# chsakell/aca-dotnet-workshop

Hardware: AMD Instinct MI355X
Metric: tasks_e2e_per_sec (higher is better)
Workload: dtype n/a (JSON over HTTP)

## Files before the change

aca_dotnet_workshop_amd/native/src/applog.hpp:

```cpp
#pragma once

#include <fcntl.h>
#include <pthread.h>
#include <sys/stat.h>
#include <unistd.h>

#include <cerrno>
#include <algorithm>
#include <atomic>
#include <chrono>
#include <condition_variable>
#include <cstdint>
#include <cstdio>
#include <cstdlib>
#include <cstring>
#include <exception>
#include <functional>
#include <future>
#include <map>
#include <mutex>
#include <stdexcept>
#include <string>
#include <string_view>
#include <thread>
#include <vector>

namespace tt {

class AppLog {
 public:
  AppLog() = default;
  AppLog(const AppLog&) = delete;
  AppLog& operator=(const AppLog&) = delete;
  ~AppLog() {
    stop_committer();
    close();
  }

  bool open(const std::string& path, int fsync_mode) {
    path_ = path;
    fsync_ = fsync_mode;
    open_fd();
    if (fsync_ == 2 && !gc_thread_.joinable()) gc_thread_ = std::thread([this] { commit_loop(); });
    return true;
  }
  bool is_open() const { return fd_ >= 0; }
  uint64_t bytes() const { return bytes_; }
  const std::string& path() const { return path_; }

  void close() {
    std::lock_guard<std::mutex> f(fd_mu_);
    if (fd_ >= 0) { ::close(fd_); fd_ = -1; }
  }

  bool group() const { return fsync_ == 2 && fd_ >= 0; }
  uint64_t mark() const { return written_.load(std::memory_order_acquire); }
  void after_durable(uint64_t mark, std::function<void()> cb) {
    if (!group() || synced_.load(std::memory_order_acquire) >= mark) {
      cb();
      return;
    }
    {
      std::lock_guard<std::mutex> l(gc_mu_);
      waiters_.emplace(mark, std::move(cb));
      gc_want_ = true;
    }
    gc_cv_.notify_one();
  }
  void wait_durable(uint64_t mark) {
    if (!group() || synced_.load(std::memory_order_acquire) >= mark) return;
    std::promise<void> done;
    auto f = done.get_future();
    after_durable(mark, [&done] { done.set_value(); });
    f.wait();
  }
  void wait_durable() { wait_durable(mark()); }
  struct CommitStats {
    uint64_t syncs, acks, written, synced;
    double sync_ms_total, sync_ms_max;
  };
  CommitStats commit_stats() {
    std::lock_guard<std::mutex> l(gc_mu_);
    return {gc_syncs_, gc_acks_, mark(), synced_.load(), gc_sync_s_ * 1e3, gc_sync_max_s_ * 1e3};
  }

  static void put_field(std::string& rec, std::string_view f) {
    uint32_t n = (uint32_t)f.size();
    rec.append(reinterpret_cast<const char*>(&n), 4);
    rec.append(f.data(), f.size());
  }
  template <class T>
  static std::string_view pod(const T& v) { return std::string_view(reinterpret_cast<const char*>(&v), sizeof(T)); }

  void append(char kind, const std::vector<std::string_view>& fields) {
    if (fd_ < 0) return;
    std::string rec;
    rec.resize(5);
    rec[4] = kind;
    for (auto f : fields) put_field(rec, f);
    uint32_t total = (uint32_t)rec.size();
    std::memcpy(&rec[0], &total, 4);
    if (batching_) {
      batch_ += rec;
      return;
    }
    write_all(rec);
  }

  class BatchScope {
   public:
    explicit BatchScope(AppLog& log) : log_(log) { log_.batching_ = true; }
    ~BatchScope() noexcept(false) {
      log_.batching_ = false;
      if (log_.batch_.empty()) return;
      std::string b;
      b.swap(log_.batch_);
      if (std::uncaught_exceptions() == 0) {
        log_.write_all(b);
        return;
      }
      try {
        log_.write_all(b);
      } catch (...) {
      }
    }
    BatchScope(const BatchScope&) = delete;
    BatchScope& operator=(const BatchScope&) = delete;

   private:
    AppLog& log_;
  };

  void replay(const std::function<void(char, std::vector<std::string_view>&)>& fn) {
    if (fd_ < 0) return;
    std::string data;
    data.resize(bytes_);
// ... 32 lines not shown
  }

  void rewrite(const std::function<void(AppLog&)>& writer) {
    if (fd_ < 0) return;
    std::string tmp = path_ + ".compact";
    AppLog out;
    ::unlink(tmp.c_str());
    out.open(tmp, 0);
    writer(out);
    ::fdatasync(out.fd_);
    out.close();
    {
      std::lock_guard<std::mutex> f(fd_mu_);
      if (::rename(tmp.c_str(), path_.c_str()) != 0) throw std::runtime_error("log compaction rename failed");
      if (fd_ >= 0) ::close(fd_);
      fd_ = -1;
      open_fd_locked();
    }
    if (fsync_ == 2) {
      {
        std::lock_guard<std::mutex> l(gc_mu_);
        gc_want_ = true;
      }
      gc_cv_.notify_one();
    }
  }

  void sync() {
    std::lock_guard<std::mutex> f(fd_mu_);
    if (fd_ >= 0) ::fdatasync(fd_);
  }

 private:
  static FILE* stall_file(double& min_s) {
    static double th = [] {
      const char* p = std::getenv("TT_STALL_MS");
      double ms = p && *p ? std::atof(p) : 100.0;
      return (ms > 0 ? ms : 100.0) / 1e3;
    }();
    static FILE* f = [] {
      const char* p = std::getenv("TT_STALL_LOG");
      return p && *p ? std::fopen(p, "a") : nullptr;
    }();
    min_s = th;
    return f;
  }

  void write_all(const std::string& rec) {
    double min_s;
    FILE* stall = stall_file(min_s);
    auto t0 = stall ? std::chrono::steady_clock::now() : std::chrono::steady_clock::time_point{};
    size_t off = 0;
    while (off < rec.size()) {
      ssize_t w = ::write(fd_, rec.data() + off, rec.size() - off);
      if (w < 0) {
        if (errno == EINTR) continue;
        throw std::runtime_error(std::string("log write failed: ") + std::strerror(errno));
      }
      off += (size_t)w;
    }
    bytes_ += rec.size();
    written_.fetch_add(rec.size(), std::memory_order_release);
    if (fsync_ == 1) ::fdatasync(fd_);
    if (stall) {
      double s = std::chrono::duration<double>(std::chrono::steady_clock::now() - t0).count();
      if (s > min_s) {
        double wall = std::chrono::duration<double>(std::chrono::system_clock::now().time_since_epoch()).count();
        std::fprintf(stall, "{\"what\": \"log-write\", \"ms\": %.2f, \"bytes\": %zu, \"log\": \"%s\", \"pid\": %d, \"wall\": %.4f}\n",
                     s * 1e3, rec.size(), path_.c_str(), (int)::getpid(), wall);
        std::fflush(stall);
      }
    }
  }

  void open_fd() {
    std::lock_guard<std::mutex> f(fd_mu_);
    open_fd_locked();
  }
  void open_fd_locked() {
    fd_ = ::open(path_.c_str(), O_RDWR | O_CREAT | O_APPEND | O_CLOEXEC, 0644);
    if (fd_ < 0) throw std::runtime_error("cannot open log " + path_ + ": " + std::strerror(errno));
// ... 33 lines not shown
      for (auto it = waiters_.begin(); it != end; ++it) ready.push_back(std::move(it->second));
      waiters_.erase(waiters_.begin(), end);
      gc_acks_ += ready.size();
      if (!waiters_.empty()) gc_want_ = true;
      l.unlock();
      for (auto& f : ready) f();
      l.lock();
    }
  }
  void stop_committer() {
    if (!gc_thread_.joinable()) return;
    {
      std::lock_guard<std::mutex> l(gc_mu_);
      gc_stop_ = true;
      gc_want_ = true;
    }
    gc_cv_.notify_one();
    gc_thread_.join();
  }

  int fd_ = -1;
  int fsync_ = 0;
  uint64_t bytes_ = 0;
  std::string path_;
  bool batching_ = false;
  std::string batch_;
  std::mutex fd_mu_;
  std::atomic<uint64_t> written_{0}, synced_{0};
  std::mutex gc_mu_;
  std::condition_variable gc_cv_;
  std::multimap<uint64_t, std::function<void()>> waiters_;
  std::thread gc_thread_;
  bool gc_stop_ = false, gc_want_ = false;
  uint64_t gc_syncs_ = 0, gc_acks_ = 0;
  double gc_sync_s_ = 0, gc_sync_max_s_ = 0;
};

}
```

aca_dotnet_workshop_amd/native/src/docstore.hpp:

```cpp
#pragma once

#include <sys/random.h>

#include <algorithm>
#include <atomic>
#include <chrono>
#include <cmath>
#include <cstdint>
#include <map>
#include <memory>
#include <mutex>
#include <optional>
#include <string>
#include <thread>
#include <unordered_map>
#include <unordered_set>
#include <vector>

#include "applog.hpp"
#include "json.hpp"
#include "shardedmap.hpp"

namespace tt {

struct EtagMismatch : std::runtime_error {
  using std::runtime_error::runtime_error;
};
struct QueryError : std::runtime_error {
  using std::runtime_error::runtime_error;
};

inline int64_t now_ms() {
  return std::chrono::duration_cast<std::chrono::milliseconds>(std::chrono::system_clock::now().time_since_epoch()).count();
}

struct Filter {
  enum Op { ALL, EQ, NEQ, GT, GTE, LT, LTE, IN, AND, OR } op = ALL;
  std::string path;
  Value val;
  std::vector<Value> vals;
  std::vector<Filter> kids;
};

inline bool ieq(std::string_view a, const char* b) {
  size_t n = std::strlen(b);
// ... 112 lines not shown
  bool disabled = false;
  uint64_t gen = 1;
  std::vector<MirrorColumn> cols;
  std::vector<std::pair<const std::string, Doc>*> nodes;
  std::vector<int64_t> seqs;
  std::vector<uint8_t> live;
  std::vector<uint32_t> kills;
  size_t live_rows = 0;
  uint64_t compactions = 0;
};

struct MirrorDelta {
  uint64_t gen = 0;
  bool on = false, disabled = false, full = false;
  size_t n = 0, from = 0, kill_cursor = 0;
  std::vector<std::string> paths;
  std::vector<size_t> dict_from;
  std::vector<std::vector<std::string>> new_values;
  std::vector<std::vector<int32_t>> ids;
  std::vector<int64_t> seqs;
  std::vector<uint8_t> live;
  std::vector<uint32_t> kills;
};

struct TxOp {
  bool is_delete = false;
  std::string key;
  std::string value;
  std::optional<std::string> etag;
  bool first_write = false;
  int64_t ttl_ms = 0;
};

class DocStore {
 public:
  explicit DocStore(const std::string& path = "", int fsync_mode = 0, size_t index_threshold = 256)
      : index_threshold_(index_threshold) {
    if (!path.empty()) {
      log_.open(path, fsync_mode);
      log_.replay([this](char kind, std::vector<std::string_view>& f) { apply_log(kind, f); });
    }
  }

  std::string set(const std::string& key, const std::string& value, const std::optional<std::string>& etag,
                  bool first_write, int64_t ttl_ms) {
    Value parsed = parse(value);
    std::string text(value);
    std::vector<Doc> graveyard;
    std::lock_guard<std::mutex> g(mu_);
    int64_t now = now_ms();
    auto it = docs_.find(key);
    check_etag_at(it, etag, first_write, now);
    it = put_at(it, key, std::move(text), std::move(parsed), ttl_ms > 0 ? now + ttl_ms : 0, &graveyard);
    log_put(key, it->second.value, it->second.etag, it->second.expire_ms);
    maybe_compact();
    return std::to_string(it->second.etag);
  }

  struct BulkItem {
    std::string key, value;
    std::optional<std::string> etag;
    bool first_write = false;
    bool have_parsed = false;
    Value parsed;
  };
  struct BulkResult {
    std::string etag;
    int err = 0;
    std::string detail;
  };
  std::vector<BulkResult> set_many(std::vector<BulkItem>& items) {
    std::vector<BulkResult> out(items.size());
    for (size_t i = 0; i < items.size(); ++i) {
      if (items[i].have_parsed) continue;
      try {
        items[i].parsed = parse(items[i].value);
      } catch (const ParseError& e) {
        out[i].err = 2;
        out[i].detail = std::string("invalid JSON: ") + e.what();
      }
    }
    std::vector<Doc> graveyard;
    graveyard.reserve(items.size());
    {
      std::lock_guard<std::mutex> g(mu_);
      {
        AppLog::BatchScope batch(log_);
        const int64_t now = now_ms();
        for (size_t i = 0; i < items.size(); ++i) {
          if (out[i].err) continue;
          BulkItem& it = items[i];
          auto dit = docs_.find(it.key);
          const bool exists = dit != docs_.end() && !expired(dit->second, now);
          if (it.etag && !it.etag->empty()) {
            if (!exists || *it.etag != std::to_string(dit->second.etag)) {
              out[i].err = 1;
              out[i].detail = "possible etag mismatch";
              continue;
            }
          } else if (it.first_write && exists) {
            out[i].err = 1;
            out[i].detail = "possible etag mismatch: first-write on existing key without etag";
            continue;
          }
          dit = put_at(dit, it.key, std::move(it.value), std::move(it.parsed), 0, &graveyard);
          log_put(it.key, dit->second.value, dit->second.etag, dit->second.expire_ms);
          out[i].etag = std::to_string(dit->second.etag);
        }
      }
      maybe_compact();
    }
    return out;
  }

  std::optional<std::pair<std::string, std::string>> get(const std::string& key) {
    std::lock_guard<std::mutex> g(mu_);
    auto it = docs_.find(key);
    if (it == docs_.end()) return std::nullopt;
    if (expired(it->second, now_ms())) { erase_locked(key, true); return std::nullopt; }
    return std::make_pair(it->second.value, std::to_string(it->second.etag));
  }

  bool del(const std::string& key, const std::optional<std::string>& etag) {
    std::lock_guard<std::mutex> g(mu_);
    auto it = docs_.find(key);
    int64_t now = now_ms();
    if (it == docs_.end() || expired(it->second, now)) {
      if (etag && !etag->empty()) throw EtagMismatch("possible etag mismatch: key not found");
      return false;
    }
    if (etag && !etag->empty() && *etag != std::to_string(it->second.etag)) throw EtagMismatch("possible etag mismatch");
    erase_locked(key, true);
    maybe_compact();
    return true;
  }

  void transact(const std::vector<TxOp>& ops) {
    std::vector<Value> parsed(ops.size());
    for (size_t i = 0; i < ops.size(); ++i)
      if (!ops[i].is_delete) parsed[i] = parse(ops[i].value);
    std::lock_guard<std::mutex> g(mu_);
    int64_t now = now_ms();
    for (auto& op : ops) {
      if (op.is_delete) {
        if (op.etag && !op.etag->empty()) {
          auto it = docs_.find(op.key);
          if (it == docs_.end() || *op.etag != std::to_string(it->second.etag)) throw EtagMismatch("possible etag mismatch in transaction");
        }
      } else {
        check_etag(op.key, op.etag, op.first_write, now);
      }
    }
    log_.append('T', {std::string_view("begin")});
    for (size_t i = 0; i < ops.size(); ++i) {
      auto& op = ops[i];
      if (op.is_delete) {
        if (docs_.count(op.key)) erase_locked(op.key, true);
      } else {
        uint64_t e = put(op.key, op.value, std::move(parsed[i]), op.ttl_ms > 0 ? now + op.ttl_ms : 0);
        log_put(op.key, op.value, e, docs_[op.key].expire_ms);
      }
    }
    log_.append('T', {std::string_view("commit")});
    maybe_compact();
  }

  static void sort_keys_to(std::string& out, std::string_view key, const Doc& d, const std::vector<std::string>& paths) {
    out += "{\"key\":";
    escape_to(out, key);
    out += ",\"etag\":\"";
    out += std::to_string(d.etag);
    out += "\",\"sort\":[";
    for (size_t j = 0; j < paths.size(); ++j) {
      if (j) out += ',';
      const Value* v = d.parsed.path(paths[j]);
      if (v) dump_to(out, *v);
      else out += "null";
    }
    out += "]}";
  }

  std::string query(const std::string& query_json, const std::string& prefix, bool sort_keys = false) {
    Value q = parse(query_json.empty() ? std::string("{}") : query_json);
    if (q.t != Value::Object) throw QueryError("query must be a JSON object");
    Filter f;
    if (auto* fv = q.get_ci("filter")) f = compile_filter(*fv);
    std::vector<SortKey> sort;
    if (auto* sv = q.get_ci("sort")) {
      if (sv->t != Value::Array) throw QueryError("sort must be an array");
      for (auto& s : sv->items) {
        const Value* k = s.get_ci("key");
        if (!k || k->t != Value::String) throw QueryError("sort entry needs a string key");
        SortKey sk{k->s, false};
        if (auto* o = s.get_ci("order")) sk.desc = o->t == Value::String && ieq(o->s, "DESC");
        sort.push_back(sk);
      }
    }
    size_t limit = 0, offset = 0;
    if (auto* pv = q.get_ci("page")) {
      if (auto* l = pv->get_ci("limit")) limit = l->t == Value::Number && l->n > 0 ? (size_t)l->n : 0;
      if (auto* t = pv->get_ci("token")) {
        if (t->t == Value::String && !t->s.empty()) offset = (size_t)std::strtoull(t->s.c_str(), nullptr, 10);
      }
    }

    std::lock_guard<std::mutex> g(mu_);
    int64_t now = now_ms();
    ensure_indexes(f);
    std::vector<std::pair<const std::string*, const Doc*>> hits;
    auto consider = [&](const std::string& key, const Doc& d) {
      if (!prefix.empty() && key.compare(0, prefix.size(), prefix) != 0) return;
      if (expired(d, now)) return;
      if (!eval_filter(f, d.parsed)) return;
      hits.emplace_back(&key, &d);
    };
    std::unordered_set<std::string> cand;
    if (candidates(f, cand)) {
      ++stats_indexed_queries_;
      for (auto& k : cand) {
        auto it = docs_.find(k);
        if (it != docs_.end()) consider(it->first, it->second);
      }
    } else {
      ++stats_scan_queries_;
      for (auto& [k, d] : docs_) consider(k, d);
    }
    if (sort.empty()) {
      std::sort(hits.begin(), hits.end(), [](auto& a, auto& b) { return a.second->seq < b.second->seq; });
    } else {
      static const Value kNull;
      std::stable_sort(hits.begin(), hits.end(), [&](auto& a, auto& b) {
        for (auto& sk : sort) {
          const Value* x = a.second->parsed.path(sk.path);
          const Value* y = b.second->parsed.path(sk.path);
          int c = compare(x ? *x : kNull, y ? *y : kNull);
          if (c) return sk.desc ? c > 0 : c < 0;
        }
        return a.second->seq < b.second->seq;
      });
    }
    size_t begin = std::min(offset, hits.size());
    size_t end = limit ? std::min(hits.size(), begin + limit) : hits.size();
    std::string out = "{\"results\":[";
    std::vector<std::string> sort_paths;
    if (sort_keys)
      for (auto& sk : sort) sort_paths.push_back(sk.path);
    for (size_t i = begin; i < end; ++i) {
      if (i > begin) out += ',';
      if (sort_keys) {
        sort_keys_to(out, std::string_view(*hits[i].first).substr(prefix.size()), *hits[i].second, sort_paths);
        continue;
      }
      out += "{\"key\":";
      escape_to(out, std::string_view(*hits[i].first).substr(prefix.size()));
      out += ",\"data\":";
      out += hits[i].second->value;
      out += ",\"etag\":\"";
      out += std::to_string(hits[i].second->etag);
      out += "\"}";
    }
    out += "]";
    if (limit && end < hits.size()) {
      out += ",\"token\":\"" + std::to_string(end) + "\"";
    }
    out += "}";
    return out;
  }

  std::vector<std::string> keys(const std::string& prefix, size_t limit) {
    std::lock_guard<std::mutex> g(mu_);
    std::vector<std::pair<uint64_t, std::string>> ks;
    int64_t now = now_ms();
    for (auto& [k, d] : docs_)
      if ((prefix.empty() || k.compare(0, prefix.size(), prefix) == 0) && !expired(d, now)) ks.emplace_back(d.seq, k);
    std::sort(ks.begin(), ks.end());
    std::vector<std::string> out;
    for (auto& p : ks) { if (limit && out.size() >= limit) break; out.push_back(p.second); }
    return out;
  }

  struct EncodedColumn {
    std::vector<std::string> values;
    std::vector<int32_t> ids;
  };
  struct Encoded {
    std::string key_blob;
    std::vector<int64_t> key_off;
    std::vector<int64_t> seqs;
    std::vector<EncodedColumn> cols;
  };
  Encoded encode_columns(const std::string& prefix, const std::vector<std::string>& paths) {
    std::lock_guard<std::mutex> g(mu_);
    int64_t now = now_ms();
    std::vector<std::pair<uint64_t, const std::pair<const std::string, Doc>*>> rows;
    rows.reserve(docs_.size());
    for (auto& kv : docs_)
      if ((prefix.empty() || kv.first.compare(0, prefix.size(), prefix) == 0) && !expired(kv.second, now))
        rows.emplace_back(kv.second.seq, &kv);
    std::sort(rows.begin(), rows.end(), [](auto& a, auto& b) { return a.first < b.first; });
    Encoded out;
    out.key_off.reserve(rows.size() + 1);
    out.seqs.reserve(rows.size());
    out.key_off.push_back(0);
    for (auto& r : rows) {
      out.key_blob += r.second->first;
      out.key_off.push_back((int64_t)out.key_blob.size());
      out.seqs.push_back((int64_t)r.first);
    }
    out.cols.resize(paths.size());
    auto encode_one = [&](size_t c) {
      const std::string& path = paths[c];
      EncodedColumn& col = out.cols[c];
      col.ids.resize(rows.size());
      std::unordered_map<std::string, int32_t> dict;
      std::string k;
      for (size_t i = 0; i < rows.size(); ++i) {
        const std::string& key = rows[i].second->first;
        const Value& doc = rows[i].second->second.parsed;
        Value tmp;
        const Value* v;
        if (path == std::string("\x00keyprefix", 10)) {
          size_t p = key.find("||");
          tmp = Value::string(p == std::string::npos ? std::string() : key.substr(0, p + 2));
          v = &tmp;
        } else if (path == std::string("\x00value", 6)) {
// ... 106 lines not shown
    if (wait > kMaxReserveS) return std::max<int64_t>(1, (int64_t)std::ceil(wait * 1000.0));
    ru_tokens_ -= ru;
    do ticket_out = next_ticket();
    while (ru_tickets_.count(ticket_out));
    Reservation res{now + wait, ru, bind};
    ru_tickets_.emplace(ticket_out, res);
    ru_by_slot_.emplace(res.slot, ticket_out);
    if (bind) ru_by_bind_.emplace(bind, ticket_out);
    return std::max<int64_t>(1, (int64_t)std::ceil(wait * 1000.0));
  }

  void debit(double ru) {
    std::lock_guard<std::mutex> g(ru_mu_);
    ru_consumed_ += ru;
    if (ru_rate_ <= 0) return;
    double now = mono_s();
    ru_tokens_ = std::min(ru_rate_, ru_tokens_ + (now - ru_last_) * ru_rate_) - ru;
    ru_last_ = now;
  }

  std::unordered_map<std::string, double> throughput_stats() {
    std::lock_guard<std::mutex> g(ru_mu_);
    return {{"ru_per_s", ru_rate_}, {"ru_consumed", ru_consumed_}, {"throttled", (double)ru_throttled_},
            {"reserved_admits", (double)ru_reserved_admits_}, {"open_reservations", (double)ru_tickets_.size()},
            {"calls", (double)ru_calls_}, {"early_retries", (double)ru_early_retries_},
            {"lapsed_reservations", (double)ru_lapsed_}, {"refunded_ru", ru_refunded_},
            {"throttled_read", (double)ru_throttled_kind_[kRead]}, {"throttled_write", (double)ru_throttled_kind_[kWrite]},
            {"throttled_query", (double)ru_throttled_kind_[kQuery]},
            {"throttled_delete", (double)ru_throttled_kind_[kDelete]},
            {"mono", mono_s()}};
  }

  bool mirror_enable(const std::vector<std::string>& paths) {
    std::lock_guard<std::mutex> g(mu_);
    if (mirror_.disabled) return false;
    std::vector<std::string> add;
    for (auto& p : paths) {
      bool have = false;
      for (auto& c : mirror_.cols) have = have || c.path == p;
      for (auto& a : add) have = have || a == p;
      if (!have) add.push_back(p);
    }
    if (mirror_.on && add.empty()) return true;
    if (!mirror_.on) {
      for (auto& [k, d] : docs_)
        if (d.expire_ms) { mirror_.disabled = true; return false; }
      mirror_.on = true;
      mirror_.cols.clear();
      for (auto& p : add) { mirror_.cols.emplace_back(); mirror_.cols.back().path = p; }
      mirror_rebuild_rows();
    } else {
      size_t first = mirror_.cols.size();
      for (auto& p : add) { mirror_.cols.emplace_back(); mirror_.cols.back().path = p; }
      auto enc = [&](size_t c) {
        MirrorColumn& col = mirror_.cols[c];
        col.ids.assign(mirror_.nodes.size(), -1);
        std::string k;
        for (size_t r = 0; r < mirror_.nodes.size(); ++r) {
          if (!mirror_.live[r]) continue;
          auto& kv = *mirror_.nodes[r];
          col.ids[r] = mirror_encode(col, kv.first, kv.second.parsed, k);
        }
      };
      parallel_for_columns(first, mirror_.cols.size(), enc);
      ++mirror_.gen;
      mirror_.kills.clear();
    }
    return true;
  }

  MirrorDelta mirror_delta(uint64_t gen, size_t from, size_t kill_from, const std::vector<size_t>& dict_sizes) {
    std::lock_guard<std::mutex> g(mu_);
    MirrorDelta d;
    d.gen = mirror_.gen;
    d.on = mirror_.on;
    d.disabled = mirror_.disabled;
    if (!mirror_.on) return d;
    size_t n = mirror_.nodes.size();
    d.full = gen != mirror_.gen || dict_sizes.size() != mirror_.cols.size() || from > n ||
             kill_from > mirror_.kills.size();
    if (d.full) from = 0, kill_from = mirror_.kills.size();
    d.n = n;
    d.from = from;
    d.kill_cursor = mirror_.kills.size();
    for (size_t i = kill_from; i < mirror_.kills.size(); ++i)
      if (mirror_.kills[i] < from) d.kills.push_back(mirror_.kills[i]);
    d.seqs.assign(mirror_.seqs.begin() + from, mirror_.seqs.end());
    d.live.assign(mirror_.live.begin() + from, mirror_.live.end());
    for (size_t c = 0; c < mirror_.cols.size(); ++c) {
      auto& col = mirror_.cols[c];
      size_t df = d.full ? 0 : std::min(dict_sizes[c], col.values.size());
      d.paths.push_back(col.path);
      d.dict_from.push_back(df);
      d.new_values.emplace_back(col.values.begin() + df, col.values.end());
      d.ids.emplace_back(col.ids.begin() + from, col.ids.end());
    }
    return d;
  }

  bool mirror_results(const int32_t* rows, size_t nrows, const std::string& prefix, const std::string& token,
                      uint64_t gen, std::string& out, size_t* skipped = nullptr,
                      const std::vector<std::string>* sort_paths = nullptr) {
    std::lock_guard<std::mutex> g(mu_);
    if (gen != mirror_.gen) return false;
    int64_t now = now_ms();
    out.clear();
    if (!sort_paths && !docs_.empty()) out.reserve(32 + token.size() + nrows * (live_bytes_ / docs_.size() + 48));
    out += "{\"results\":[";
    size_t skip = 0;
    bool first = true;
    for (size_t i = 0; i < nrows; ++i) {
      uint32_t r = (uint32_t)rows[i];
      if (r >= mirror_.nodes.size() || !mirror_.live[r]) { ++skip; continue; }
      auto* it = mirror_.nodes[r];
      const std::string& key = it->first;
      if (it->second.mrow != r || expired(it->second, now)) { ++skip; continue; }
      if (!first) out += ',';
      first = false;
      if (sort_paths) {
        sort_keys_to(out, std::string_view(key).substr(std::min(prefix.size(), key.size())), it->second, *sort_paths);
        continue;
      }
      out += "{\"key\":";
      escape_to(out, std::string_view(key).substr(std::min(prefix.size(), key.size())));
      out += ",\"data\":";
      out += it->second.value;
      out += ",\"etag\":\"";
      out += std::to_string(it->second.etag);
      out += "\"}";
    }
    out += "]";
    if (!token.empty()) out += ",\"token\":\"" + token + "\"";
    out += "}";
    if (skipped) *skipped = skip;
    return true;
  }

  std::unordered_map<std::string, uint64_t> mirror_stats() {
    std::lock_guard<std::mutex> g(mu_);
    return {{"on", mirror_.on}, {"disabled", mirror_.disabled}, {"gen", mirror_.gen},
            {"rows", mirror_.nodes.size()}, {"live_rows", mirror_.live_rows}, {"columns", mirror_.cols.size()},
            {"compactions", mirror_.compactions}};
  }

  size_t size() {
    std::lock_guard<std::mutex> g(mu_);
    return docs_.size();
  }

  void compact() {
    std::lock_guard<std::mutex> g(mu_);
    compact_locked();
  }

  void sync() { std::lock_guard<std::mutex> g(mu_); log_.sync(); }
  bool group_commit() const { return log_.group(); }
  uint64_t log_mark() const { return log_.mark(); }
  void after_durable(uint64_t mark, std::function<void()> cb) { log_.after_durable(mark, std::move(cb)); }
  void wait_durable() { log_.wait_durable(); }
  AppLog::CommitStats commit_stats() { return log_.commit_stats(); }

  std::unordered_map<std::string, uint64_t> stats() {
    std::lock_guard<std::mutex> g(mu_);
    return {{"docs", docs_.size()}, {"live_bytes", live_bytes_}, {"log_bytes", log_.bytes()},
            {"indexes", indexes_.size()}, {"indexed_queries", stats_indexed_queries_},
            {"scan_queries", stats_scan_queries_}, {"etag", etag_}};
  }

  std::vector<std::string> indexed_paths() {
    std::lock_guard<std::mutex> g(mu_);
    std::vector<std::string> out;
    for (auto& [p, _] : indexes_) out.push_back(p);
    std::sort(out.begin(), out.end());
    return out;
  }

 private:
  using Index = std::unordered_map<std::string, std::unordered_set<std::string>>;
  using Docs = ShardedMap<Doc>;

  static bool expired(const Doc& d, int64_t now) { return d.expire_ms && d.expire_ms <= now; }

  void check_etag(const std::string& key, const std::optional<std::string>& etag, bool first_write, int64_t now) {
    check_etag_at(docs_.find(key), etag, first_write, now);
  }

  void check_etag_at(Docs::iterator it, const std::optional<std::string>& etag,
                     bool first_write, int64_t now) {
    bool exists = it != docs_.end() && !expired(it->second, now);
    if (etag && !etag->empty()) {
      if (!exists || *etag != std::to_string(it->second.etag)) throw EtagMismatch("possible etag mismatch");
    } else if (first_write && exists) {
      throw EtagMismatch("possible etag mismatch: first-write on existing key without etag");
    }
  }

  uint64_t put(const std::string& key, const std::string& value, Value parsed, int64_t expire_ms) {
    return put_at(docs_.find(key), key, std::string(value), std::move(parsed), expire_ms, nullptr)->second.etag;
  }

  static bool same_scalar(const Value* a, const Value* b) {
    if (!a || !b) return a == b;
    if (a->t != b->t) return false;
    switch (a->t) {
      case Value::Null: return true;
      case Value::Bool: return a->b == b->b;
      case Value::Number: return std::memcmp(&a->n, &b->n, sizeof(double)) == 0;
      case Value::String: return a->s == b->s;
      default: return false;
    }
  }

  Docs::iterator put_at(Docs::iterator it,
                                                       const std::string& key, std::string&& value, Value parsed,
                                                       int64_t expire_ms, std::vector<Doc>* graveyard) {
    uint64_t e = ++etag_;
    if (expire_ms && mirror_.on) mirror_disable();
    int32_t* reuse = nullptr;
    if (it == docs_.end()) {
      Doc d;
      live_bytes_ += key.size() + value.size();
      d.value = std::move(value);
      d.parsed = std::move(parsed);
      d.etag = e;
      d.seq = ++seq_;
      d.expire_ms = expire_ms;
      index_add(key, d.parsed);
      it = docs_.emplace(key, std::move(d)).first;
    } else {
      Doc& d = it->second;
      index_update(key, d.parsed, parsed);
      if (mirror_.on && d.mrow < mirror_.live.size() && mirror_.live[d.mrow]) {
        reuse_.resize(mirror_.cols.size());
        for (size_t c = 0; c < mirror_.cols.size(); ++c)
          reuse_[c] = same_column_value(mirror_.cols[c], d.parsed, parsed) ? mirror_.cols[c].ids[d.mrow] : kEncode;
        reuse = reuse_.data();
      }
      live_bytes_ += value.size();
      live_bytes_ -= d.value.size();
      if (graveyard) {
        graveyard->emplace_back();
        graveyard->back().value.swap(d.value);
        graveyard->back().parsed = std::move(d.parsed);
// ... 39 lines not shown
      erase_locked(std::string(f[0]), false);
    }
  }

  void maybe_compact() {
    if (!log_.is_open()) return;
    uint64_t live = live_bytes_ + docs_.size() * 40;
    if (log_.bytes() > (1u << 20) && log_.bytes() > 4 * live) compact_locked();
  }

  void compact_locked() {
    if (!log_.is_open()) return;
    std::vector<std::pair<uint64_t, const std::pair<const std::string, Doc>*>> rows;
    for (auto& kv : docs_) rows.emplace_back(kv.second.seq, &kv);
    std::sort(rows.begin(), rows.end(), [](auto& a, auto& b) { return a.first < b.first; });
    log_.rewrite([&](AppLog& out) {
      for (auto& r : rows)
        out.append('P', {r.second->first, r.second->second.value, AppLog::pod(r.second->second.etag),
                         AppLog::pod(r.second->second.expire_ms)});
    });
  }

  template <class F>
  void parallel_for_columns(size_t lo, size_t hi, F&& f) {
    if (hi - lo <= 1 || mirror_.nodes.size() < 100000) {
      for (size_t c = lo; c < hi; ++c) f(c);
      return;
    }
    std::vector<std::thread> ts;
    for (size_t c = lo; c < hi; ++c) ts.emplace_back(f, c);
    for (auto& t : ts) t.join();
  }

  static int32_t mirror_encode(MirrorColumn& col, const std::string& key, const Value& doc, std::string& k) {
    static const std::string kPrefix("\x00keyprefix", 10), kValue("\x00value", 6);
    Value tmp;
    const Value* v;
    if (col.path == kPrefix) {
      size_t p = key.find("||");
      tmp = Value::string(p == std::string::npos ? std::string() : key.substr(0, p + 2));
      v = &tmp;
    } else if (col.path == kValue) {
      v = doc.t == Value::Object ? nullptr : &doc;
    } else {
      v = doc.path(col.path);
    }
    if (!v) return -1;
    mirror_key(*v, k);
    auto it = col.dict.find(k);
    if (it == col.dict.end()) {
      it = col.dict.emplace(k, (int32_t)col.values.size()).first;
      col.values.push_back(dump(*v));
    }
    return it->second;
  }

  static bool same_column_value(const MirrorColumn& col, const Value& before, const Value& after) {
    static const std::string kPrefix("\x00keyprefix", 10), kValue("\x00value", 6);
    if (col.path == kPrefix) return true;
    if (col.path == kValue)
      return before.t != Value::Object && after.t != Value::Object && same_scalar(&before, &after);
    return same_scalar(before.path(col.path), after.path(col.path));
  }

  void mirror_append(std::pair<const std::string, Doc>& kv, const int32_t* reuse = nullptr) {
    uint32_t r = (uint32_t)mirror_.nodes.size();
    mirror_.nodes.push_back(&kv);
    mirror_.seqs.push_back((int64_t)kv.second.seq);
    mirror_.live.push_back(1);
    std::string k;
    for (size_t c = 0; c < mirror_.cols.size(); ++c) {
      MirrorColumn& col = mirror_.cols[c];
      col.ids.push_back(reuse && reuse[c] != kEncode ? reuse[c] : mirror_encode(col, kv.first, kv.second.parsed, k));
    }
    kv.second.mrow = r;
    ++mirror_.live_rows;
    if (mirror_.nodes.size() > 65536 && mirror_.nodes.size() > 2 * mirror_.live_rows) mirror_compact();
  }

  void mirror_kill(Doc& d) {
    if (d.mrow == UINT32_MAX) return;
    if (mirror_.on && d.mrow < mirror_.live.size() && mirror_.live[d.mrow]) {
      mirror_.live[d.mrow] = 0;
      mirror_.kills.push_back(d.mrow);
      --mirror_.live_rows;
    }
    d.mrow = UINT32_MAX;
  }

  void mirror_disable() {
    for (auto& kv : docs_) kv.second.mrow = UINT32_MAX;
    uint64_t gen = mirror_.gen;
    mirror_ = ColumnMirror{};
    mirror_.gen = gen + 1;
    mirror_.disabled = true;
  }

  void mirror_rebuild_rows() {
    std::vector<std::pair<uint64_t, std::pair<const std::string, Doc>*>> rows;
    rows.reserve(docs_.size());
    for (auto& kv : docs_) rows.emplace_back(kv.second.seq, &kv);
    std::sort(rows.begin(), rows.end(), [](auto& a, auto& b) { return a.first < b.first; });
    mirror_.nodes.clear();
    mirror_.seqs.clear();
    mirror_.kills.clear();
    mirror_.nodes.reserve(rows.size());
    for (auto& r : rows) {
// ... 11 lines not shown
        col.ids[i] = mirror_encode(col, rows[i].second->first, rows[i].second->second.parsed, k);
    };
    parallel_for_columns(0, mirror_.cols.size(), enc);
    ++mirror_.gen;
  }

  void mirror_compact() {
    size_t w = 0, n = mirror_.nodes.size();
    for (size_t r = 0; r < n; ++r) {
      if (!mirror_.live[r]) continue;
      if (w != r) {
        mirror_.nodes[w] = mirror_.nodes[r];
        mirror_.seqs[w] = mirror_.seqs[r];
        for (auto& col : mirror_.cols) col.ids[w] = col.ids[r];
        mirror_.nodes[w]->second.mrow = (uint32_t)w;
      }
      ++w;
    }
    mirror_.nodes.resize(w);
    mirror_.seqs.resize(w);
    for (auto& col : mirror_.cols) col.ids.resize(w);
    mirror_.live.assign(w, 1);
    mirror_.live_rows = w;
    mirror_.kills.clear();
    ++mirror_.gen;
    ++mirror_.compactions;
  }

  void collect_eq_paths(const Filter& f, std::vector<std::string>& out) {
    if (f.op == Filter::EQ || f.op == Filter::IN) out.push_back(f.path);
    for (auto& k : f.kids) collect_eq_paths(k, out);
  }

  void ensure_indexes(const Filter& f) {
    if (docs_.size() < index_threshold_) return;
    std::vector<std::string> paths;
    collect_eq_paths(f, paths);
    for (auto& p : paths) {
      if (indexes_.count(p)) continue;
      Index& idx = indexes_[p];
      for (auto& [k, d] : docs_) {
        const Value* v = d.parsed.path(p);
        if (v && v->t != Value::Array && v->t != Value::Object) idx[index_key(*v)].insert(k);
      }
    }
  }

  void index_add(const std::string& key, const Value& doc) {
    for (auto& [p, idx] : indexes_) {
      const Value* v = doc.path(p);
      if (v && v->t != Value::Array && v->t != Value::Object) idx[index_key(*v)].insert(key);
    }
  }

  void index_update(const std::string& key, const Value& before, const Value& after) {
    for (auto& [p, idx] : indexes_) {
      const Value* a = before.path(p);
      const Value* b = after.path(p);
      if (same_scalar(a, b)) continue;
      if (a && a->t != Value::Array && a->t != Value::Object) {
        auto it = idx.find(index_key(*a));
        if (it != idx.end()) {
          it->second.erase(key);
          if (it->second.empty()) idx.erase(it);
        }
      }
// ... 23 lines not shown
        return true;
      }
      case Filter::IN: {
        auto ix = indexes_.find(f.path);
        if (ix == indexes_.end()) return false;
        for (auto& v : f.vals) {
          if (v.t == Value::Array || v.t == Value::Object) return false;
          auto it = ix->second.find(index_key(v));
          if (it != ix->second.end()) out.insert(it->second.begin(), it->second.end());
        }
        return true;
      }
      case Filter::AND: {
        bool any = false;
        std::unordered_set<std::string> best;
        for (auto& k : f.kids) {
          std::unordered_set<std::string> c;
          if (candidates(k, c) && (!any || c.size() < best.size())) { best.swap(c); any = true; }
        }
        if (any) out.insert(best.begin(), best.end());
        return any;
      }
      case Filter::OR: {
        std::unordered_set<std::string> acc;
        for (auto& k : f.kids)
          if (!candidates(k, acc)) return false;
        out.insert(acc.begin(), acc.end());
        return true;
      }
      default: return false;
    }
  }

  std::mutex mu_;
  Docs docs_;
  std::unordered_map<std::string, Index> indexes_;
  AppLog log_;
  uint64_t etag_ = 0;
  uint64_t seq_ = 0;
  uint64_t live_bytes_ = 0;
  uint64_t stats_indexed_queries_ = 0;
  uint64_t stats_scan_queries_ = 0;
  size_t index_threshold_;
  ColumnMirror mirror_;
  static constexpr int32_t kEncode = INT32_MIN;
  std::vector<int32_t> reuse_;
  std::mutex ru_mu_;
  std::atomic<bool> ru_on_{false};
  double ru_rate_ = 0, ru_tokens_ = 0, ru_last_ = 0, ru_consumed_ = 0;
  uint64_t ru_throttled_ = 0, ru_reserved_admits_ = 0, ru_calls_ = 0, ru_early_retries_ = 0, ru_lapsed_ = 0;
  uint64_t ru_throttled_kind_[4] = {0, 0, 0, 0};
  double ru_refunded_ = 0;
  double ru_ticket_ttl_s_ = kTicketTtlS;
  struct Reservation {
    double slot, ru;
    uint64_t bind;
  };
  std::unordered_map<uint64_t, Reservation> ru_tickets_;
  std::multimap<double, uint64_t> ru_by_slot_;
  std::unordered_multimap<uint64_t, uint64_t> ru_by_bind_;
  uint64_t ru_rng_[2] = {0, 0};
  uint64_t next_ticket() {
    if ((ru_rng_[0] | ru_rng_[1]) == 0) {
      if (getrandom(ru_rng_, sizeof ru_rng_, 0) != (ssize_t)sizeof ru_rng_ || (ru_rng_[0] | ru_rng_[1]) == 0)
        ru_rng_[0] = 0x9e3779b97f4a7c15ull ^ (uint64_t)(mono_s() * 1e9);
    }
    uint64_t a = ru_rng_[0];
    const uint64_t b = ru_rng_[1];
    ru_rng_[0] = b;
    a ^= a << 23;
    ru_rng_[1] = a ^ b ^ (a >> 17) ^ (b >> 26);
    uint64_t v = (ru_rng_[1] + b) >> 1;
    return v ? v : 1;
  }
  void drop(std::unordered_map<uint64_t, Reservation>::iterator it) {
// ... 36 lines not shown
```

Before: 87220.

## Replace store mutex with rwlock and split bulk writes into shared prepare and exclusive commit

The document store's mutex becomes a writer-preferring pthread rwlock. Reads (get, queries with existing indexes, mirror results, stats) take a shared lock, and set_many now precomputes index ops, mirror column ids and encoded log records under shared locks in slices. The exclusive section then only applies the prepared plan, falling back to the old path when a version or shape has changed. Mirror result emission gains prefetching, and the log gets an append-encoded path. This aims to cut time spent holding the exclusive lock, at the cost of more complexity, double lookups and rwlock overhead on short critical sections.

Measured after the change: 87140. Within noise of the previous version (-0.1%).

```diff
diff --git a/aca_dotnet_workshop_amd/native/src/applog.hpp b/aca_dotnet_workshop_amd/native/src/applog.hpp
--- a/aca_dotnet_workshop_amd/native/src/applog.hpp
+++ b/aca_dotnet_workshop_amd/native/src/applog.hpp
@@ -56,7 +56,7 @@
   bool group() const { return fsync_ == 2 && fd_ >= 0; }
   uint64_t mark() const { return written_.load(std::memory_order_acquire); }
   void after_durable(uint64_t mark, std::function<void()> cb) {
-    if (!group() || synced_.load(std::memory_order_acquire) >= mark) {
+    if (!group() || covered(mark)) {
       cb();
       return;
     }
@@ -68,7 +68,7 @@
     gc_cv_.notify_one();
   }
   void wait_durable(uint64_t mark) {
-    if (!group() || synced_.load(std::memory_order_acquire) >= mark) return;
+    if (!group() || covered(mark)) return;
     std::promise<void> done;
     auto f = done.get_future();
     after_durable(mark, [&done] { done.set_value(); });
@@ -81,7 +81,7 @@
   };
   CommitStats commit_stats() {
     std::lock_guard<std::mutex> l(gc_mu_);
-    return {gc_syncs_, gc_acks_, mark(), synced_.load(), gc_sync_s_ * 1e3, gc_sync_max_s_ * 1e3};
+    return {gc_syncs_, gc_acks_.load(), mark(), synced_.load(), gc_sync_s_ * 1e3, gc_sync_max_s_ * 1e3};
   }
 
   static void put_field(std::string& rec, std::string_view f) {
@@ -92,16 +92,27 @@
   template <class T>
   static std::string_view pod(const T& v) { return std::string_view(reinterpret_cast<const char*>(&v), sizeof(T)); }
 
+  static size_t encode(std::string& out, char kind, const std::vector<std::string_view>& fields) {
+    const size_t at = out.size();
+    out.resize(at + 5);
+    out[at + 4] = kind;
+    for (auto f : fields) put_field(out, f);
+    uint32_t total = (uint32_t)(out.size() - at);
+    std::memcpy(&out[at], &total, 4);
+    return at;
+  }
+
   void append(char kind, const std::vector<std::string_view>& fields) {
     if (fd_ < 0) return;
     std::string rec;
-    rec.resize(5);
-    rec[4] = kind;
-    for (auto f : fields) put_field(rec, f);
-    uint32_t total = (uint32_t)rec.size();
-    std::memcpy(&rec[0], &total, 4);
+    encode(rec, kind, fields);
+    append_encoded(rec);
+  }
+
+  void append_encoded(std::string_view rec) {
+    if (fd_ < 0) return;
     if (batching_) {
-      batch_ += rec;
+      batch_.append(rec.data(), rec.size());
       return;
     }
     write_all(rec);
@@ -200,6 +211,12 @@
   }
 
  private:
+  bool covered(uint64_t mark) {
+    if (synced_.load(std::memory_order_acquire) < mark) return false;
+    gc_acks_.fetch_add(1, std::memory_order_relaxed);
+    return true;
+  }
+
   static FILE* stall_file(double& min_s) {
     static double th = [] {
       const char* p = std::getenv("TT_STALL_MS");
@@ -214,7 +231,7 @@
     return f;
   }
 
-  void write_all(const std::string& rec) {
+  void write_all(std::string_view rec) {
     double min_s;
     FILE* stall = stall_file(min_s);
     auto t0 = stall ? std::chrono::steady_clock::now() : std::chrono::steady_clock::time_point{};
@@ -314,7 +331,8 @@
   std::multimap<uint64_t, std::function<void()>> waiters_;
   std::thread gc_thread_;
   bool gc_stop_ = false, gc_want_ = false;
-  uint64_t gc_syncs_ = 0, gc_acks_ = 0;
+  uint64_t gc_syncs_ = 0;
+  std::atomic<uint64_t> gc_acks_{0};
   double gc_sync_s_ = 0, gc_sync_max_s_ = 0;
 };
 
diff --git a/aca_dotnet_workshop_amd/native/src/docstore.hpp b/aca_dotnet_workshop_amd/native/src/docstore.hpp
--- a/aca_dotnet_workshop_amd/native/src/docstore.hpp
+++ b/aca_dotnet_workshop_amd/native/src/docstore.hpp
@@ -1,5 +1,6 @@
 #pragma once
 
+#include <pthread.h>
 #include <sys/random.h>
 
 #include <algorithm>
@@ -7,10 +8,12 @@
 #include <chrono>
 #include <cmath>
 #include <cstdint>
+#include <functional>
 #include <map>
 #include <memory>
 #include <mutex>
 #include <optional>
+#include <shared_mutex>
 #include <string>
 #include <thread>
 #include <unordered_map>
@@ -189,7 +192,33 @@
   int64_t ttl_ms = 0;
 };
 
+class RwLock {
+ public:
+  RwLock() {
+    pthread_rwlockattr_t a;
+    pthread_rwlockattr_init(&a);
+#ifdef PTHREAD_RWLOCK_PREFER_WRITER_NONRECURSIVE_NP
+    pthread_rwlockattr_setkind_np(&a, PTHREAD_RWLOCK_PREFER_WRITER_NONRECURSIVE_NP);
+#endif
+    pthread_rwlock_init(&l_, &a);
+    pthread_rwlockattr_destroy(&a);
+  }
+  ~RwLock() { pthread_rwlock_destroy(&l_); }
+  RwLock(const RwLock&) = delete;
+  RwLock& operator=(const RwLock&) = delete;
+  void lock() { pthread_rwlock_wrlock(&l_); }
+  void unlock() { pthread_rwlock_unlock(&l_); }
+  void lock_shared() { pthread_rwlock_rdlock(&l_); }
+  void unlock_shared() { pthread_rwlock_unlock(&l_); }
+
+ private:
+  pthread_rwlock_t l_;
+};
+
 class DocStore {
+  using Exclusive = std::lock_guard<RwLock>;
+  using Shared = std::shared_lock<RwLock>;
+
  public:
   explicit DocStore(const std::string& path = "", int fsync_mode = 0, size_t index_threshold = 256)
       : index_threshold_(index_threshold) {
@@ -204,7 +233,7 @@
     Value parsed = parse(value);
     std::string text(value);
     std::vector<Doc> graveyard;
-    std::lock_guard<std::mutex> g(mu_);
+    Exclusive g(mu_);
     int64_t now = now_ms();
     auto it = docs_.find(key);
     check_etag_at(it, etag, first_write, now);
@@ -227,51 +256,93 @@
     std::string detail;
   };
   std::vector<BulkResult> set_many(std::vector<BulkItem>& items) {
+    using clk = std::chrono::steady_clock;
+    auto ns = [](clk::time_point a, clk::time_point b) {
+      return (uint64_t)std::chrono::duration_cast<std::chrono::nanoseconds>(b - a).count();
+    };
     std::vector<BulkResult> out(items.size());
-    for (size_t i = 0; i < items.size(); ++i) {
-      if (items[i].have_parsed) continue;
-      try {
-        items[i].parsed = parse(items[i].value);
-      } catch (const ParseError& e) {
-        out[i].err = 2;
-        out[i].detail = std::string("invalid JSON: ") + e.what();
-      }
-    }
+    parse_items(items, out);
+    std::vector<Doc> graveyard;
+    graveyard.reserve(items.size());
+    std::vector<uint64_t> etags(items.size(), 0);
+    BulkPlan plan;
+    uint64_t prepare_ns = 0;
+    for (size_t from = 0; from < items.size(); from += kPrepareSlice) {
+      Shared s(mu_);
+      const auto t0 = clk::now();
+      const bool go_on = prepare_bulk(items, out, plan, from, std::min(items.size(), from + kPrepareSlice));
+      prepare_ns += ns(t0, clk::now());
+      if (!go_on) break;
+    }
+    bulk_prepare_us_.fetch_add(prepare_ns / 1000, std::memory_order_relaxed);
+    if (bulk_gap_hook_) bulk_gap_hook_();
+    {
+      Exclusive g(mu_);
+      const auto t0 = clk::now();
+      {
+        AppLog::BatchScope batch(log_);
+        const int64_t now = now_ms();
+        const bool same_shape = plan.mirror_on == mirror_.on && plan.ncols == mirror_.cols.size() &&
+                                plan.nindexes == indexes_.size();
+        uint64_t prepared = 0, fallback = 0;
+        for (size_t i = 0; i < items.size(); ++i) {
+          if (out[i].err) continue;
+          ++prepared;
+          auto dit = docs_.find(items[i].key);
+          const uint64_t version = dit == docs_.end() ? 0 : dit->second.etag;
+          if (same_shape && version == plan.items[i].seen) {
+            etags[i] = commit_prepared(dit, items[i], out[i], plan, i, now, graveyard);
+          } else {
+            ++fallback;
+            etags[i] = bulk_put_locked(dit, items[i], out[i], now, graveyard);
+          }
+        }
+        bulk_prepared_.fetch_add(prepared, std::memory_order_relaxed);
+        bulk_fallback_.fetch_add(fallback, std::memory_order_relaxed);
+      }
+      maybe_compact();
+      bulk_hold_us_.fetch_add(ns(t0, clk::now()) / 1000, std::memory_order_relaxed);
+    }
+    for (size_t i = 0; i < items.size(); ++i)
+      if (etags[i]) out[i].etag = std::to_string(etags[i]);
+    return out;
+  }
+
+  std::vector<BulkResult> set_many_serial(std::vector<BulkItem>& items) {
+    std::vector<BulkResult> out(items.size());
+    parse_items(items, out);
     std::vector<Doc> graveyard;
     graveyard.reserve(items.size());
     {
-      std::lock_guard<std::mutex> g(mu_);
+      Exclusive g(mu_);
+      const auto t0 = std::chrono::steady_clock::now();
       {
         AppLog::BatchScope batch(log_);
         const int64_t now = now_ms();
         for (size_t i = 0; i < items.size(); ++i) {
           if (out[i].err) continue;
-          BulkItem& it = items[i];
-          auto dit = docs_.find(it.key);
-          const bool exists = dit != docs_.end() && !expired(dit->second, now);
-          if (it.etag && !it.etag->empty()) {
-            if (!exists || *it.etag != std::to_string(dit->second.etag)) {
-              out[i].err = 1;
-              out[i].detail = "possible etag mismatch";
-              continue;
-            }
-          } else if (it.first_write && exists) {
-            out[i].err = 1;
-            out[i].detail = "possible etag mismatch: first-write on existing key without etag";
-            continue;
-          }
-          dit = put_at(dit, it.key, std::move(it.value), std::move(it.parsed), 0, &graveyard);
-          log_put(it.key, dit->second.value, dit->second.etag, dit->second.expire_ms);
-          out[i].etag = std::to_string(dit->second.etag);
+          if (uint64_t e = bulk_put_locked(docs_.find(items[i].key), items[i], out[i], now, graveyard))
+            out[i].etag = std::to_string(e);
         }
       }
       maybe_compact();
+      bulk_hold_us_.fetch_add(
+          (uint64_t)std::chrono::duration_cast<std::chrono::microseconds>(std::chrono::steady_clock::now() - t0).count(),
+          std::memory_order_relaxed);
     }
     return out;
   }
 
+  void set_bulk_gap_hook(std::function<void()> hook) { bulk_gap_hook_ = std::move(hook); }
+
   std::optional<std::pair<std::string, std::string>> get(const std::string& key) {
-    std::lock_guard<std::mutex> g(mu_);
+    {
+      Shared s(mu_);
+      auto it = docs_.find(key);
+      if (it == docs_.end()) return std::nullopt;
+      if (!expired(it->second, now_ms())) return std::make_pair(it->second.value, std::to_string(it->second.etag));
+    }
+    Exclusive g(mu_);
     auto it = docs_.find(key);
     if (it == docs_.end()) return std::nullopt;
     if (expired(it->second, now_ms())) { erase_locked(key, true); return std::nullopt; }
@@ -279,7 +350,7 @@
   }
 
   bool del(const std::string& key, const std::optional<std::string>& etag) {
-    std::lock_guard<std::mutex> g(mu_);
+    Exclusive g(mu_);
     auto it = docs_.find(key);
     int64_t now = now_ms();
     if (it == docs_.end() || expired(it->second, now)) {
@@ -296,7 +367,7 @@
     std::vector<Value> parsed(ops.size());
     for (size_t i = 0; i < ops.size(); ++i)
       if (!ops[i].is_delete) parsed[i] = parse(ops[i].value);
-    std::lock_guard<std::mutex> g(mu_);
+    Exclusive g(mu_);
     int64_t now = now_ms();
     for (auto& op : ops) {
       if (op.is_delete) {
@@ -361,9 +432,19 @@
       }
     }
 
-    std::lock_guard<std::mutex> g(mu_);
+    {
+      Shared s(mu_);
+      if (!missing_index(f)) return query_locked(f, sort, limit, offset, prefix, sort_keys);
+    }
+    Exclusive g(mu_);
+    ensure_indexes(f);
+    return query_locked(f, sort, limit, offset, prefix, sort_keys);
+  }
+
+ private:
+  std::string query_locked(const Filter& f, const std::vector<SortKey>& sort, size_t limit, size_t offset,
+                           const std::string& prefix, bool sort_keys) {
     int64_t now = now_ms();
-    ensure_indexes(f);
     std::vector<std::pair<const std::string*, const Doc*>> hits;
     auto consider = [&](const std::string& key, const Doc& d) {
       if (!prefix.empty() && key.compare(0, prefix.size(), prefix) != 0) return;
@@ -373,13 +454,13 @@
     };
     std::unordered_set<std::string> cand;
     if (candidates(f, cand)) {
-      ++stats_indexed_queries_;
+      stats_indexed_queries_.fetch_add(1, std::memory_order_relaxed);
       for (auto& k : cand) {
         auto it = docs_.find(k);
         if (it != docs_.end()) consider(it->first, it->second);
       }
     } else {
-      ++stats_scan_queries_;
+      stats_scan_queries_.fetch_add(1, std::memory_order_relaxed);
       for (auto& [k, d] : docs_) consider(k, d);
     }
     if (sort.empty()) {
@@ -424,8 +505,9 @@
     return out;
   }
 
+ public:
   std::vector<std::string> keys(const std::string& prefix, size_t limit) {
-    std::lock_guard<std::mutex> g(mu_);
+    Exclusive g(mu_);
     std::vector<std::pair<uint64_t, std::string>> ks;
     int64_t now = now_ms();
     for (auto& [k, d] : docs_)
@@ -447,7 +529,7 @@
     std::vector<EncodedColumn> cols;
   };
   Encoded encode_columns(const std::string& prefix, const std::vector<std::string>& paths) {
-    std::lock_guard<std::mutex> g(mu_);
+    Exclusive g(mu_);
     int64_t now = now_ms();
     std::vector<std::pair<uint64_t, const std::pair<const std::string, Doc>*>> rows;
     rows.reserve(docs_.size());
@@ -620,7 +702,7 @@
   }
 
   bool mirror_enable(const std::vector<std::string>& paths) {
-    std::lock_guard<std::mutex> g(mu_);
+    Exclusive g(mu_);
     if (mirror_.disabled) return false;
     std::vector<std::string> add;
     for (auto& p : paths) {
@@ -658,7 +740,7 @@
   }
 
   MirrorDelta mirror_delta(uint64_t gen, size_t from, size_t kill_from, const std::vector<size_t>& dict_sizes) {
-    std::lock_guard<std::mutex> g(mu_);
+    Shared g(mu_);
     MirrorDelta d;
     d.gen = mirror_.gen;
     d.on = mirror_.on;
@@ -689,7 +771,7 @@
   bool mirror_results(const int32_t* rows, size_t nrows, const std::string& prefix, const std::string& token,
                       uint64_t gen, std::string& out, size_t* skipped = nullptr,
                       const std::vector<std::string>* sort_paths = nullptr) {
-    std::lock_guard<std::mutex> g(mu_);
+    Shared g(mu_);
     if (gen != mirror_.gen) return false;
     int64_t now = now_ms();
     out.clear();
@@ -697,7 +779,16 @@
     out += "{\"results\":[";
     size_t skip = 0;
     bool first = true;
+    constexpr size_t kAhead = 8;
+    auto live_node = [&](size_t i) -> const std::pair<const std::string, Doc>* {
+      uint32_t r = (uint32_t)rows[i];
+      return r < mirror_.nodes.size() && mirror_.live[r] ? mirror_.nodes[r] : nullptr;
+    };
     for (size_t i = 0; i < nrows; ++i) {
+      if (i + kAhead < nrows)
+        if (auto* n = live_node(i + kAhead)) __builtin_prefetch(&n->second);
+      if (i + kAhead / 2 < nrows)
+        if (auto* n = live_node(i + kAhead / 2)) __builtin_prefetch(n->second.value.data());
       uint32_t r = (uint32_t)rows[i];
       if (r >= mirror_.nodes.size() || !mirror_.live[r]) { ++skip; continue; }
       auto* it = mirror_.nodes[r];
@@ -725,23 +816,23 @@
   }
 
   std::unordered_map<std::string, uint64_t> mirror_stats() {
-    std::lock_guard<std::mutex> g(mu_);
+    Shared g(mu_);
     return {{"on", mirror_.on}, {"disabled", mirror_.disabled}, {"gen", mirror_.gen},
             {"rows", mirror_.nodes.size()}, {"live_rows", mirror_.live_rows}, {"columns", mirror_.cols.size()},
             {"compactions", mirror_.compactions}};
   }
 
   size_t size() {
-    std::lock_guard<std::mutex> g(mu_);
+    Shared g(mu_);
     return docs_.size();
   }
 
   void compact() {
-    std::lock_guard<std::mutex> g(mu_);
+    Exclusive g(mu_);
     compact_locked();
   }
 
-  void sync() { std::lock_guard<std::mutex> g(mu_); log_.sync(); }
+  void sync() { Exclusive g(mu_); log_.sync(); }
   bool group_commit() const { return log_.group(); }
   uint64_t log_mark() const { return log_.mark(); }
   void after_durable(uint64_t mark, std::function<void()> cb) { log_.after_durable(mark, std::move(cb)); }
@@ -749,14 +840,16 @@
   AppLog::CommitStats commit_stats() { return log_.commit_stats(); }
 
   std::unordered_map<std::string, uint64_t> stats() {
-    std::lock_guard<std::mutex> g(mu_);
+    Shared g(mu_);
     return {{"docs", docs_.size()}, {"live_bytes", live_bytes_}, {"log_bytes", log_.bytes()},
-            {"indexes", indexes_.size()}, {"indexed_queries", stats_indexed_queries_},
-            {"scan_queries", stats_scan_queries_}, {"etag", etag_}};
+            {"indexes", indexes_.size()}, {"indexed_queries", stats_indexed_queries_.load()},
+            {"scan_queries", stats_scan_queries_.load()}, {"etag", etag_},
+            {"bulk_prepared", bulk_prepared_.load()}, {"bulk_fallback", bulk_fallback_.load()},
+            {"bulk_hold_us", bulk_hold_us_.load()}, {"bulk_prepare_us", bulk_prepare_us_.load()}};
   }
 
   std::vector<std::string> indexed_paths() {
-    std::lock_guard<std::mutex> g(mu_);
+    Exclusive g(mu_);
     std::vector<std::string> out;
     for (auto& [p, _] : indexes_) out.push_back(p);
     std::sort(out.begin(), out.end());
@@ -797,6 +890,209 @@
       case Value::String: return a->s == b->s;
       default: return false;
     }
+  }
+
+  static void parse_items(std::vector<BulkItem>& items, std::vector<BulkResult>& out) {
+    for (size_t i = 0; i < items.size(); ++i) {
+      if (items[i].have_parsed) continue;
+      try {
+        items[i].parsed = parse(items[i].value);
+      } catch (const ParseError& e) {
+        out[i].err = 2;
+        out[i].detail = std::string("invalid JSON: ") + e.what();
+      }
+    }
+  }
+
+  static void bulk_precondition_failed(const BulkItem& it, BulkResult& r) {
+    r.err = 1;
+    r.detail = it.etag && !it.etag->empty() ? "possible etag mismatch"
+                                            : "possible etag mismatch: first-write on existing key without etag";
+  }
+
+  uint64_t bulk_put_locked(Docs::iterator dit, BulkItem& it, BulkResult& r, int64_t now, std::vector<Doc>& graveyard) {
+    const bool exists = dit != docs_.end() && !expired(dit->second, now);
+    const bool has_etag = it.etag && !it.etag->empty();
+    if (has_etag ? (!exists || *it.etag != std::to_string(dit->second.etag)) : (it.first_write && exists)) {
+      bulk_precondition_failed(it, r);
+      return 0;
+    }
+    dit = put_at(dit, it.key, std::move(it.value), std::move(it.parsed), 0, &graveyard);
+    log_put(it.key, dit->second.value, dit->second.etag, dit->second.expire_ms);
+    return dit->second.etag;
+  }
+
+  struct PreparedColumn {
+    int32_t id = kEncode;
+    std::string key, text;
+  };
+  struct IndexOp {
+    Index* index;
+    bool add;
+    std::string value;
+  };
+  struct PreparedItem {
+    uint64_t seen = 0;
+    bool etag_match = false;
+    int64_t bytes = 0;
+    size_t ops_from = 0, ops_to = 0;
+    size_t rec_at = 0, rec_len = 0;
+  };
+  struct BulkPlan {
+    bool mirror_on = false;
+    size_t ncols = 0, nindexes = 0;
+    std::vector<PreparedItem> items;
+    std::vector<PreparedColumn> cols;
+    std::vector<IndexOp> ops;
+    std::string log;
+  };
+  static constexpr size_t kPrepareSlice = 16;
+  static constexpr size_t kRecEtagFromEnd = 20;
+
+  static bool indexable(const Value* v) { return v && v->t != Value::Array && v->t != Value::Object; }
+
+  bool prepare_bulk(const std::vector<BulkItem>& items, const std::vector<BulkResult>& out, BulkPlan& plan,
+                    size_t from, size_t to) {
+    const size_t n = items.size();
+    const bool logging = log_.is_open();
+    if (from == 0) {
+      plan.mirror_on = mirror_.on;
+      plan.ncols = mirror_.cols.size();
+      plan.nindexes = indexes_.size();
+      plan.items.resize(n);
+      if (plan.mirror_on) plan.cols.resize(n * plan.ncols);
+      if (logging) {
+        size_t log_bytes = 0;
+        for (size_t i = 0; i < n; ++i)
+          if (!out[i].err) log_bytes += items[i].key.size() + items[i].value.size() + 37;
+        plan.log.reserve(log_bytes);
+      }
+    } else if (plan.mirror_on != mirror_.on || plan.ncols != mirror_.cols.size() || plan.nindexes != indexes_.size()) {
+      plan.nindexes = SIZE_MAX;
+      return false;
+    }
+    std::string k;
+    const uint64_t etag0 = 0;
+    const int64_t expire0 = 0;
+    for (size_t i = from; i < to; ++i) {
+      if (out[i].err) continue;
+      const BulkItem& it = items[i];
+      PreparedItem& p = plan.items[i];
+      auto dit = docs_.find(it.key);
+      const Doc* old = dit != docs_.end() ? &dit->second : nullptr;
+      p.ops_from = plan.ops.size();
+      if (old) {
+        p.seen = old->etag;
+        p.etag_match = it.etag && !it.etag->empty() && *it.etag == std::to_string(old->etag);
+        p.bytes = (int64_t)it.value.size() - (int64_t)old->value.size();
+        for (auto& [path, idx] : indexes_) {
+          const Value* a = old->parsed.path(path);
+          const Value* b = it.parsed.path(path);
+          if (same_scalar(a, b)) continue;
+          if (indexable(a)) plan.ops.push_back({&idx, false, index_key(*a)});
+          if (indexable(b)) plan.ops.push_back({&idx, true, index_key(*b)});
+        }
+      } else {
+        p.bytes = (int64_t)(it.key.size() + it.value.size());
+        for (auto& [path, idx] : indexes_) {
+          const Value* b = it.parsed.path(path);
+          if (indexable(b)) plan.ops.push_back({&idx, true, index_key(*b)});
+        }
+      }
+      p.ops_to = plan.ops.size();
+      if (plan.mirror_on) {
+        PreparedColumn* pc = &plan.cols[i * plan.ncols];
+        const bool carry = old && old->mrow < mirror_.live.size() && mirror_.live[old->mrow];
+        for (size_t c = 0; c < plan.ncols; ++c) {
+          MirrorColumn& col = mirror_.cols[c];
+          if (carry && same_column_value(col, old->parsed, it.parsed)) {
+            pc[c].id = col.ids[old->mrow];
+            continue;
+          }
+          Value tmp;
+          const Value* v = mirror_value(col, it.key, it.parsed, tmp);
+          if (!v) {
+            pc[c].id = -1;
+            continue;
+          }
+          mirror_key(*v, k);
+          auto f = col.dict.find(k);
+          if (f != col.dict.end()) {
+            pc[c].id = f->second;
+          } else {
+            pc[c].key = k;
+            pc[c].text = dump(*v);
+          }
+        }
+      }
+      if (logging) {
+        p.rec_at = AppLog::encode(plan.log, 'P', {it.key, it.value, AppLog::pod(etag0), AppLog::pod(expire0)});
+        p.rec_len = plan.log.size() - p.rec_at;
+      }
+    }
+    return true;
+  }
+
+  uint64_t commit_prepared(Docs::iterator dit, BulkItem& it, BulkResult& r, BulkPlan& plan, size_t i, int64_t now,
+                           std::vector<Doc>& graveyard) {
+    PreparedItem& p = plan.items[i];
+    const bool found = dit != docs_.end();
+    const bool exists = found && !expired(dit->second, now);
+    const bool has_etag = it.etag && !it.etag->empty();
+    if (has_etag ? (!exists || !p.etag_match) : (it.first_write && exists)) {
+      bulk_precondition_failed(it, r);
+      return 0;
+    }
+    const uint64_t e = ++etag_;
+    for (size_t o = p.ops_from; o < p.ops_to; ++o) {
+      IndexOp& op = plan.ops[o];
+      if (op.add) {
+        (*op.index)[op.value].insert(it.key);
+      } else {
+        auto f = op.index->find(op.value);
+        if (f != op.index->end()) {
+          f->second.erase(it.key);
+          if (f->second.empty()) op.index->erase(f);
+        }
+      }
+    }
+    live_bytes_ += (uint64_t)p.bytes;
+    if (!found) {
+      Doc d;
+      d.value = std::move(it.value);
+      d.parsed = std::move(it.parsed);
+      d.etag = e;
+      d.seq = ++seq_;
+      dit = docs_.emplace(it.key, std::move(d)).first;
+    } else {
+      Doc& d = dit->second;
+      graveyard.emplace_back();
+      graveyard.back().value.swap(d.value);
+      graveyard.back().parsed = std::move(d.parsed);
+      d.value = std::move(it.value);
+      d.parsed = std::move(it.parsed);
+      d.etag = e;
+      d.expire_ms = 0;
+      mirror_kill(d);
+    }
+    if (mirror_.on) {
+      PreparedColumn* pc = &plan.cols[i * plan.ncols];
+      mirror_append_ids(*dit, [&](size_t c) {
+        if (pc[c].id != kEncode) return pc[c].id;
+        MirrorColumn& col = mirror_.cols[c];
+        auto f = col.dict.find(pc[c].key);
+        if (f == col.dict.end()) {
+          f = col.dict.emplace(pc[c].key, (int32_t)col.values.size()).first;
+          col.values.push_back(std::move(pc[c].text));
+        }
+        return f->second;
+      });
+    }
+    if (p.rec_len) {
+      std::memcpy(&plan.log[p.rec_at + p.rec_len - kRecEtagFromEnd], &e, sizeof e);
+      log_.append_encoded(std::string_view(plan.log).substr(p.rec_at, p.rec_len));
+    }
+    return e;
   }
 
   Docs::iterator put_at(Docs::iterator it,
@@ -902,19 +1198,20 @@
     for (auto& t : ts) t.join();
   }
 
-  static int32_t mirror_encode(MirrorColumn& col, const std::string& key, const Value& doc, std::string& k) {
+  static const Value* mirror_value(const MirrorColumn& col, const std::string& key, const Value& doc, Value& tmp) {
     static const std::string kPrefix("\x00keyprefix", 10), kValue("\x00value", 6);
-    Value tmp;
-    const Value* v;
     if (col.path == kPrefix) {
       size_t p = key.find("||");
       tmp = Value::string(p == std::string::npos ? std::string() : key.substr(0, p + 2));
-      v = &tmp;
-    } else if (col.path == kValue) {
-      v = doc.t == Value::Object ? nullptr : &doc;
-    } else {
-      v = doc.path(col.path);
-    }
+      return &tmp;
+    }
+    if (col.path == kValue) return doc.t == Value::Object ? nullptr : &doc;
+    return doc.path(col.path);
+  }
+
+  static int32_t mirror_encode(MirrorColumn& col, const std::string& key, const Value& doc, std::string& k) {
+    Value tmp;
+    const Value* v = mirror_value(col, key, doc, tmp);
     if (!v) return -1;
     mirror_key(*v, k);
     auto it = col.dict.find(k);
@@ -934,15 +1231,19 @@
   }
 
   void mirror_append(std::pair<const std::string, Doc>& kv, const int32_t* reuse = nullptr) {
+    std::string k;
+    mirror_append_ids(kv, [&](size_t c) {
+      return reuse && reuse[c] != kEncode ? reuse[c] : mirror_encode(mirror_.cols[c], kv.first, kv.second.parsed, k);
+    });
+  }
+
+  template <class F>
+  void mirror_append_ids(std::pair<const std::string, Doc>& kv, F&& id_of) {
     uint32_t r = (uint32_t)mirror_.nodes.size();
     mirror_.nodes.push_back(&kv);
     mirror_.seqs.push_back((int64_t)kv.second.seq);
     mirror_.live.push_back(1);
-    std::string k;
-    for (size_t c = 0; c < mirror_.cols.size(); ++c) {
-      MirrorColumn& col = mirror_.cols[c];
-      col.ids.push_back(reuse && reuse[c] != kEncode ? reuse[c] : mirror_encode(col, kv.first, kv.second.parsed, k));
-    }
+    for (size_t c = 0; c < mirror_.cols.size(); ++c) mirror_.cols[c].ids.push_back(id_of(c));
     kv.second.mrow = r;
     ++mirror_.live_rows;
     if (mirror_.nodes.size() > 65536 && mirror_.nodes.size() > 2 * mirror_.live_rows) mirror_compact();
@@ -1020,6 +1321,15 @@
     for (auto& k : f.kids) collect_eq_paths(k, out);
   }
 
+  bool missing_index(const Filter& f) {
+    if (docs_.size() < index_threshold_) return false;
+    std::vector<std::string> paths;
+    collect_eq_paths(f, paths);
+    for (auto& p : paths)
+      if (!indexes_.count(p)) return true;
+    return false;
+  }
+
   void ensure_indexes(const Filter& f) {
     if (docs_.size() < index_threshold_) return;
     std::vector<std::string> paths;
@@ -1109,15 +1419,17 @@
     }
   }
 
-  std::mutex mu_;
+  RwLock mu_;
+  std::function<void()> bulk_gap_hook_;
+  std::atomic<uint64_t> bulk_prepared_{0}, bulk_fallback_{0}, bulk_hold_us_{0}, bulk_prepare_us_{0};
   Docs docs_;
   std::unordered_map<std::string, Index> indexes_;
   AppLog log_;
   uint64_t etag_ = 0;
   uint64_t seq_ = 0;
   uint64_t live_bytes_ = 0;
-  uint64_t stats_indexed_queries_ = 0;
-  uint64_t stats_scan_queries_ = 0;
+  std::atomic<uint64_t> stats_indexed_queries_{0};
+  std::atomic<uint64_t> stats_scan_queries_{0};
   size_t index_threshold_;
   ColumnMirror mirror_;
   static constexpr int32_t kEncode = INT32_MIN;
```
